# dawn-search/dawnsearch

Measured on NVIDIA B200. Metric: queries/sec, exact top-k over N x 384 fp16, higher is better.
Workload: dtype s8 x s8 -> s32 filter on an int8 shadow (tensor cores) / f32 scan, exact f32 re-score over the fp16 rows

## Files before the change

dawnsearch_b200/csrc/dawn_common.cuh:

```cuda
#pragma once

#include <cuda_fp16.h>
#include <cuda_runtime.h>
#include <stdint.h>

namespace dawn {

constexpr int kDim = 384;
constexpr int kRowBytesF16 = kDim * 2;
constexpr int kMaxCand = 128;
constexpr int kI8BlockRows = 8;
constexpr int kI8BlockBytes = kI8BlockRows * kDim + kI8BlockRows * 4;
constexpr uint32_t kNoRow = 0xFFFFFFFFu;
constexpr uint64_t kNoLabel = 0xFFFFFFFFFFFFFFFFull;

struct __align__(16) Cand {
    float score;
    uint32_t row;
    uint64_t label;
};

__host__ __device__ inline Cand empty_cand() {
    Cand c;
#ifdef __CUDA_ARCH__
    c.score = __int_as_float(0xff800000);
#else
    c.score = -__builtin_inff();
#endif
    c.row = kNoRow;
    c.label = kNoLabel;
    return c;
}

__host__ __device__ inline bool cand_better(const Cand &a, const Cand &b) {
    if (a.score != b.score) return a.score > b.score;
    if (a.label != b.label) return a.label < b.label;
    return a.row < b.row;
}

__device__ inline uint32_t float_to_ordered(float f) {
    uint32_t u = __float_as_uint(f);
    return (u & 0x80000000u) ? ~u : (u | 0x80000000u);
}
__device__ inline float ordered_to_float(uint32_t u) {
    return __uint_as_float((u & 0x80000000u) ? (u & 0x7FFFFFFFu) : ~u);
}

__host__ __device__ inline uint64_t mix64(uint64_t z) {
    z = (z ^ (z >> 30)) * 0xBF58476D1CE4E5B9ull;
    z = (z ^ (z >> 27)) * 0x94D049BB133111EBull;
    return z ^ (z >> 31);
}
__host__ __device__ inline int32_t synth_raw(uint64_t seed, uint64_t row, uint32_t col) {
    uint64_t h = mix64(seed + 0x9E3779B97F4A7C15ull * (row * (uint64_t)kDim + col + 1));
    uint32_t s = (uint32_t)(h & 0xFFFF) + (uint32_t)((h >> 16) & 0xFFFF) +
                 (uint32_t)((h >> 32) & 0xFFFF) + (uint32_t)(h >> 48);
    return (int32_t)s - 131070;
}


cudaError_t launch_ingest_f16(const float *src_f32, __half *dst, size_t n_rows, cudaStream_t s);
cudaError_t launch_synth_f16(__half *dst, uint64_t seed, uint64_t first_row, size_t n_rows,
                             cudaStream_t s);
cudaError_t launch_synth_f32(float *dst, uint64_t seed, uint64_t first_row, size_t n_rows, cudaStream_t s);
cudaError_t launch_gather_f32(const __half *corpus, const uint32_t *rows, size_t n, float *out,
                              cudaStream_t s);
cudaError_t launch_iota_labels(uint64_t *dst, uint64_t first, size_t n, cudaStream_t s);
cudaError_t launch_shadow_quantize(const __half *corpus, uint8_t *arena, size_t first, size_t n, uint32_t *kappa_bits, cudaStream_t s);
cudaError_t launch_truncate_by_limit(const float *dist, uint32_t *counts, size_t batch, size_t k, float limit, cudaStream_t s);

struct ScanLaunch {
    const __half *corpus;
    const uint64_t *labels;
    uint32_t n_rows;
    const float *queries;
    int nq;
    int kprime;
    Cand *partials;
    uint32_t *chunk_counter;
    uint32_t *status;
    int grid;
    float score_floor;
};
cudaError_t launch_scan_topk_f16(const ScanLaunch &p, cudaStream_t s);
int scan_max_queries_per_pass(int kprime);

struct FinalizeLaunch {
    const __half *corpus;
    const float *queries;
    int nq;
    const Cand *partials;
    int n_lists;
    int kprime;
    int k;
    float eps;
    uint64_t *labels_out;
    float *distances_out;
    uint32_t *counts_out;
    uint32_t *flags_out;
    int scalar;
    const float *corpus32;
    const float *eps_q;
    const uint32_t *overflow;
    uint32_t *counters;
    int n_counters;
    uint32_t *status_out;
    float eps_scale;
    uint32_t *stats;
};
cudaError_t launch_score_error(const uint2 *log, const uint32_t *cnt, int n_queries, int log_cap, const __half *corpus,
                               const float *q32, const __half *q16, const float *eps_q, unsigned long long *out,
                               cudaStream_t s);
cudaError_t launch_finalize(const FinalizeLaunch &p, cudaStream_t s);

struct __align__(16) I8Query {
    int8_t hi[kDim];
    int8_t lo[kDim];
    float s1, s2;
    float pad_[2];
};
__host__ __device__ inline size_t i8_row_offset(size_t row) {
// ... 90 lines not shown
```

dawnsearch_b200/csrc/dawn_index.cu:

```cuda
#include <atomic>
#include <cmath>
#include <cstdarg>
#include <cstdio>
#include <cstdlib>
#include <cstring>
#include <chrono>
#include <condition_variable>
#include <mutex>
#include <new>
#include <shared_mutex>
#include <string>
#include <thread>
#include <vector>

#include "../../include/dawn_index.h"
#include "dawn_common.cuh"

using namespace dawn;

namespace {

thread_local std::string g_last_error;

int fail(int code, const char *fmt, ...) {
// ... 72 lines not shown
    std::shared_mutex corpus_mu;
    int device = 0;
    int sm_count = 0;
    cudaStream_t stream = nullptr;
    std::atomic<bool> dead{false};

    int scalar = DAWN_SCALAR_F16;
    __half *corpus = nullptr;
    float *corpus32 = nullptr;
    uint64_t *labels = nullptr;
    std::atomic<uint8_t *> shadow{nullptr};
    std::atomic<size_t> shadow_rows{0};
    std::atomic<float> shadow_kappa{0.f};
    uint32_t *d_shadow_kappa = nullptr;
    std::atomic<size_t> size{0};
    std::atomic<size_t> capacity{0};
    size_t phys = 0;

    float *h_stage_buf[2] = {nullptr, nullptr};
    uint64_t *h_labels_buf[2] = {nullptr, nullptr};
    float *d_stage_buf[2] = {nullptr, nullptr};
    cudaEvent_t stage_done[2] = {nullptr, nullptr};
    bool stage_busy[2] = {false, false};
    int stage_cur = 0;
    float *h_stage = nullptr;
    uint64_t *h_stage_labels = nullptr;
    std::atomic<size_t> staged{0};
    float *d_stage = nullptr;
    BulkLane bulk[kBulkThreads];
    bool bulk_ready = false;

    uint32_t *d_norm_stats = nullptr;
    uint32_t *h_norm_stats = nullptr;
    size_t norm_checked = 0;
    uint64_t bad_rows = 0;
    float norm_max = 0.f, norm_min = INFINITY;

    uint32_t *d_stats = nullptr;
    uint32_t *h_stats = nullptr;

    std::atomic<int64_t> gemm_min_batch{16};
    std::atomic<int64_t> gemm_min_rows{65536};
    std::atomic<int64_t> gemm_small_batch{2};
    std::atomic<int64_t> gemm_small_batch_rows{2000000};
    std::atomic<int64_t> force_path{0};
    std::atomic<int64_t> gemm_cta_group{0};
    std::atomic<int64_t> gemm_chunk_tiles{0};
    std::atomic<int64_t> gemm_sequential_tiles{0};
    std::atomic<int64_t> gemm_growth{0};
    std::atomic<int64_t> gemm_unit_sync{1};
    std::atomic<int64_t> i8_tensor_min_batch{16};
    std::atomic<int64_t> i8_tensor_chunk_rows{4 << 20};
    std::atomic<int64_t> shadow_i8{0};
    std::atomic<int64_t> shadow_big_k_rows{40000000};
    std::atomic<int64_t> shadow_single_rows{6000000};
    std::atomic<int64_t> i8_native{1};

    std::mutex pool_mu;
    std::condition_variable pool_cv;
    std::vector<SearchWs *> pool_free;
    int pool_total = 0;
    std::mutex dev_mu;
    SearchWs *dev_ws = nullptr;

    std::atomic<bool> profiling{false};
    std::mutex prof_mu;
    dawn_profile prof{};
};

namespace {

#define CK(idx, expr)                                                                         \
    do {                                                                                      \
        cudaError_t e__ = (expr);                                                             \
        if (e__ != cudaSuccess) {                                                             \
            (idx)->dead = true;                                                               \
            return fail(DAWN_ERR_CUDA, "%s failed: %s (%s:%d)", #expr, cudaGetErrorString(e__), \
                        __FILE__, __LINE__);                                                  \
        }                                                                                     \
    } while (0)

int check_alive(dawn_index *idx) {
    if (!idx) return fail(DAWN_ERR_INVALID, "null index handle");
    if (idx->dead) return fail(DAWN_ERR_CUDA, "index is in a failed state after an earlier CUDA error");
    cudaError_t e = cudaSetDevice(idx->device);
    if (e != cudaSuccess) {
        idx->dead = true;
        return fail(DAWN_ERR_CUDA, "cudaSetDevice(%d): %s", idx->device, cudaGetErrorString(e));
    }
    return DAWN_OK;
}


void free_ws(SearchWs *ws) {
    if (!ws) return;
    if (ws->stream) cudaStreamSynchronize(ws->stream);
    for (auto &p : ws->pending) ws->free_events.push_back(p);
    for (auto &p : ws->free_events) {
        cudaEventDestroy(p.a);
        cudaEventDestroy(p.b);
    }
    cudaFree(ws->d_queries);
    cudaFreeHost(ws->h_queries);
    cudaFree(ws->d_result);
    cudaFreeHost(ws->h_result);
    cudaFree(ws->d_i8_scratch);
// ... 239 lines not shown
    if (idx->norm_checked >= n) return DAWN_OK;
    CK(idx, launch_verify_rows(idx->corpus, idx->scalar == DAWN_SCALAR_I8 ? 1 : 0, idx->norm_checked, n - idx->norm_checked, idx->d_norm_stats, idx->stream));
    CK(idx, cudaMemcpyAsync(idx->h_norm_stats, idx->d_norm_stats, 4 * sizeof(uint32_t), cudaMemcpyDeviceToHost, idx->stream));
    CK(idx, cudaStreamSynchronize(idx->stream));
    idx->bad_rows = idx->h_norm_stats[0];
    memcpy(&idx->norm_max, &idx->h_norm_stats[1], 4);
    uint32_t inv = ~idx->h_norm_stats[2];
    memcpy(&idx->norm_min, &inv, 4);
    idx->norm_checked = n;
    return DAWN_OK;
}

inline float eps_scale_of(const dawn_index *idx) {
    return idx->norm_max > kRowNormGate ? idx->norm_max / 1.01f * 1.001f : 1.0f;
}

void reset_norm_stats(dawn_index *idx) {
    const uint32_t init[4] = {0u, 0u, 0u, 0u};
    cudaMemcpyAsync(idx->d_norm_stats, init, sizeof init, cudaMemcpyHostToDevice, idx->stream);
    cudaStreamSynchronize(idx->stream);
    idx->norm_checked = 0;
    idx->bad_rows = 0;
    idx->norm_max = 0.f;
    idx->norm_min = INFINITY;
}

void drop_shadow(dawn_index *idx) {
    uint8_t *p = idx->shadow.exchange(nullptr);
    if (p) cudaFree(p);
    idx->shadow_rows = 0;
    idx->shadow_kappa = 0.f;
}

int ensure_shadow(dawn_index *idx) {
    if (!idx->shadow_i8 || idx->scalar != DAWN_SCALAR_F16) return DAWN_OK;
    const size_t n = idx->size;
    if (n < 65536 || idx->shadow_rows >= n) return DAWN_OK;
    if (!idx->shadow) {
        const size_t bytes = (idx->phys + kI8BlockRows - 1) / kI8BlockRows * (size_t)kI8BlockBytes;
        uint8_t *p = nullptr;
        if (cudaMalloc(&p, bytes) != cudaSuccess || (!idx->d_shadow_kappa && cudaMalloc(&idx->d_shadow_kappa, 4) != cudaSuccess)) {
            cudaGetLastError();
            if (p) cudaFree(p);
            idx->shadow_i8 = 0;
            return DAWN_OK;
        }
        CK(idx, cudaMemsetAsync(p, 0, bytes, idx->stream));
        CK(idx, cudaMemsetAsync(idx->d_shadow_kappa, 0, 4, idx->stream));
        idx->shadow = p;
        idx->shadow_rows = 0;
        idx->shadow_kappa = 0.f;
    }
    const size_t first = idx->shadow_rows;
    CK(idx, launch_shadow_quantize(idx->corpus, idx->shadow, first, n - first, idx->d_shadow_kappa, idx->stream));
    uint32_t bits = 0;
    CK(idx, cudaMemcpyAsync(&bits, idx->d_shadow_kappa, 4, cudaMemcpyDeviceToHost, idx->stream));
    CK(idx, cudaStreamSynchronize(idx->stream));
    float kappa;
    memcpy(&kappa, &bits, 4);
    idx->shadow_kappa = kappa * 1.0001f + 1e-4f;
    idx->shadow_rows = n;
    return DAWN_OK;
}

bool debug_stages() {
    static const bool on = getenv("DAWN_DEBUG_STAGES") != nullptr;
    return on;
}
void debug_wait(SearchWs *ws, cudaStream_t s, const char *stage) {
    if (!debug_stages()) return;
    const auto t0 = std::chrono::steady_clock::now();
    while (true) {
        cudaError_t e = cudaStreamQuery(s);
        if (e == cudaSuccess) {
            fprintf(stderr, "[dawn debug] %s done\n", stage);
            return;
        }
        if (e != cudaErrorNotReady) {
            fprintf(stderr, "[dawn debug] %s: %s\n", stage, cudaGetErrorString(e));
            return;
        }
        if (std::chrono::duration<double>(std::chrono::steady_clock::now() - t0).count() > 5.0) {
            uint32_t c[4] = {0, 0, 0, 0};
            cudaStream_t side;
            cudaStreamCreateWithFlags(&side, cudaStreamNonBlocking);
            if (ws->d_counters) {
                cudaMemcpyAsync(c, ws->d_counters, sizeof(c), cudaMemcpyDeviceToHost, side);
                cudaStreamSynchronize(side);
            }
            fprintf(stderr, "[dawn debug] %s STILL RUNNING after 5 s (rows %zu, counters %u %u %u %u)\n", stage, ws->n_rows, c[0],
                    c[1], c[2], c[3]);
            fflush(stderr);
            return;
        }
    }
}

int choose_kprime(size_t k) {
    size_t want = k + (k / 8 > 4 ? k / 8 : 4);
    int kp = 16;
    while ((size_t)kp < want) kp <<= 1;
    return kp > kMaxCand ? kMaxCand : kp;
}

struct ResultView {
    uint64_t *labels;
    float *dist;
// ... 1207 lines not shown
    gs.final_lists = nullptr;
    gs.accum_slack = kGemmAccumSlack;
    gs.limit_score = -INFINITY;
    gs.debug_raw_scores = 1;
    const float *eps_q = nullptr;
    const uint2 *log = nullptr;
    const uint32_t *cnt = nullptr;
    const __half *q16 = nullptr;
    gs.eps_out = &eps_q;
    gs.debug_log_out = &log;
    gs.debug_cnt_out = &cnt;
    gs.debug_q16_out = &q16;
    CK(idx, launch_gemm_search(gs, s));
    unsigned long long *d_out = nullptr;
    CK(idx, cudaMalloc(&d_out, 48 * sizeof(unsigned long long)));
    CK(idx, cudaMemsetAsync(d_out, 0, 48 * sizeof(unsigned long long), s));
    CK(idx, launch_score_error(log, cnt, (int)batch, 2048, idx->corpus, ws->d_queries, q16, eps_q, d_out, s));
    unsigned long long h[48];
    CK(idx, cudaMemcpyAsync(h, d_out, sizeof h, cudaMemcpyDeviceToHost, s));
    CK(idx, cudaStreamSynchronize(s));
    cudaFree(d_out);
    auto as_double = [](unsigned long long u) { double d; memcpy(&d, &u, 8); return d; };
    auto upd = [](double &a, double b) { if (b > a) a = b; };
    upd(acc->max_mma_vs_f64, as_double(h[0]));
    upd(acc->max_seq_vs_f64, as_double(h[1]));
    upd(acc->max_mma_vs_seq, as_double(h[2]));
    upd(acc->max_err_over_eps_q, as_double(h[3]));
    acc->pairs += h[4];
    for (int b = 0; b < 40; b++) acc->hist[b] += h[8 + b];
    acc->scan_eps = kScanEps;
    acc->gemm_accum_slack = kGemmAccumSlack;
    acc->i8_dequant_slack = kI8DequantSlack;
    return DAWN_OK;
}

int dawn_index_set_option(dawn_index *idx, const char *key, int64_t value) {
    int rc = check_alive(idx);
    if (rc) return rc;
    if (!key) return fail(DAWN_ERR_INVALID, "key is null");
    if (!strcmp(key, "gemm_min_batch")) idx->gemm_min_batch = value;
    else if (!strcmp(key, "gemm_min_rows")) idx->gemm_min_rows = value;
    else if (!strcmp(key, "gemm_small_batch")) idx->gemm_small_batch = value;
    else if (!strcmp(key, "gemm_small_batch_rows")) idx->gemm_small_batch_rows = value;
    else if (!strcmp(key, "force_path")) idx->force_path = value;
    else if (!strcmp(key, "gemm_cta_group")) idx->gemm_cta_group = value;
    else if (!strcmp(key, "gemm_chunk_tiles")) idx->gemm_chunk_tiles = value;
    else if (!strcmp(key, "gemm_sequential_tiles")) idx->gemm_sequential_tiles = value;
    else if (!strcmp(key, "gemm_growth")) idx->gemm_growth = value;
    else if (!strcmp(key, "gemm_unit_sync")) idx->gemm_unit_sync = value;
    else if (!strcmp(key, "i8_tensor_min_batch")) idx->i8_tensor_min_batch = value;
    else if (!strcmp(key, "i8_tensor_chunk_rows")) idx->i8_tensor_chunk_rows = value < 65536 ? 65536 : value;
    else if (!strcmp(key, "i8_native")) idx->i8_native = value;
    else if (!strcmp(key, "shadow_i8")) idx->shadow_i8 = value;
    else if (!strcmp(key, "shadow_single_rows")) idx->shadow_single_rows = value;
    else if (!strcmp(key, "shadow_big_k_rows")) idx->shadow_big_k_rows = value;
    else return fail(DAWN_ERR_INVALID, "unknown option '%s'", key);
    return DAWN_OK;
}

int dawn_index_set_profiling(dawn_index *idx, int enable) {
    int rc = check_alive(idx);
    if (rc) return rc;
    {
        std::lock_guard<std::mutex> lk(idx->dev_mu);
        drain_events(idx->dev_ws, idx->dev_ws->ws_used ? idx->dev_ws->ws_stream : idx->dev_ws->stream);
        merge_profile(idx, idx->dev_ws);
    }
    idx->profiling = enable != 0;
    return DAWN_OK;
}

int dawn_index_get_profile(dawn_index *idx, dawn_profile *out, int reset) {
    int rc = check_alive(idx);
    if (rc) return rc;
    if (!out) return fail(DAWN_ERR_INVALID, "out is null");
    {
        std::lock_guard<std::mutex> lk(idx->dev_mu);
        SearchWs *ws = idx->dev_ws;
        cudaStream_t s = ws->ws_used ? ws->ws_stream : ws->stream;
        drain_events(ws, s);
        merge_profile(idx, ws);
        if (ws->ws_used) CK(idx, cudaEventSynchronize(ws->ws_done));
        CK(idx, cudaMemcpy(idx->h_stats, idx->d_stats, 4 * sizeof(uint32_t), cudaMemcpyDeviceToHost));
        if (reset) CK(idx, cudaMemset(idx->d_stats, 0, 4 * sizeof(uint32_t)));
    }
    std::lock_guard<std::mutex> lk(idx->prof_mu);
    *out = idx->prof;
    out->device_uncertified = idx->h_stats[0];
    out->device_status = idx->h_stats[1];
    {
        float e;
        memcpy(&e, &idx->h_stats[2], 4);
        out->max_selection_error = e;
    }
    if (reset) idx->prof = dawn_profile{};
    return DAWN_OK;
}

int dawn_merge_results_device(int device, const uint64_t *d_labels, const float *d_distances,
                              const uint32_t *d_counts, size_t n_lists, size_t list_stride_bytes,
                              size_t batch, size_t k, uint64_t *d_labels_out, float *d_distances_out,
                              uint32_t *d_counts_out, void *stream) {
    if (!d_labels || !d_distances || !d_counts || !d_labels_out || !d_distances_out || !d_counts_out)
        return fail(DAWN_ERR_INVALID, "null device pointer");
    if (k == 0 || k > DAWN_MAX_K || n_lists == 0 || n_lists * k > 1024)
        return fail(DAWN_ERR_INVALID, "merge shape out of range (n_lists=%zu k=%zu; n_lists*k must be <= 1024)",
// ... 163 lines not shown
        if (finite) {
            vmax = fmaxf(vmax, len);
            vmin = fminf(vmin, len);
        }
    }
    if (lane == 0) {
        if (bad) atomicAdd(&stats[0], bad);
        atomicMax(&stats[1], __float_as_uint(vmax));
        atomicMax(&stats[2], ~__float_as_uint(vmin));
    }
}

__global__ void __launch_bounds__(256) iota_labels_kernel(uint64_t *__restrict__ dst, uint64_t first, size_t n) {
    size_t stride = (size_t)gridDim.x * blockDim.x;
    for (size_t i = (size_t)blockIdx.x * blockDim.x + threadIdx.x; i < n; i += stride) dst[i] = first + i;
}

cudaError_t launch_merge_results(const uint64_t *labels, const float *dist, const uint32_t *counts, int n_lists,
                                 size_t list_stride_bytes, int batch, int k, uint64_t *labels_out, float *dist_out,
                                 uint32_t *counts_out, cudaStream_t s) {
    if (n_lists > 64) return cudaErrorInvalidValue;
    size_t sl = list_stride_bytes, sd = list_stride_bytes, sc = list_stride_bytes;
    if (list_stride_bytes == 0) {
        sl = (size_t)batch * k * sizeof(uint64_t);
        sd = (size_t)batch * k * sizeof(float);
        sc = (size_t)batch * sizeof(uint32_t);
    }
    merge_results_kernel<<<batch, 1024, 0, s>>>(labels, dist, counts, n_lists, sl, sd, sc, batch, k, labels_out,
                                                dist_out, counts_out);
    return cudaGetLastError();
}

cudaError_t launch_find_label(const uint64_t *labels, size_t n, uint64_t label, uint32_t *row_out,
                              cudaStream_t s) {
    cudaError_t e = cudaMemsetAsync(row_out, 0xFF, sizeof(uint32_t), s);
    if (e != cudaSuccess) return e;
    size_t blocks = (n + 255) / 256;
    if (blocks > 148 * 8) blocks = 148 * 8;
    find_label_kernel<<<(unsigned)blocks, 256, 0, s>>>(labels, n, label, row_out);
    return cudaGetLastError();
}

cudaError_t launch_verify_rows(const void *arena, int scalar, size_t first, size_t n, uint32_t *stats, cudaStream_t s) {
    if (n == 0) return cudaSuccess;
    size_t blocks = (n + 7) / 8;
    if (blocks > 148 * 8) blocks = 148 * 8;
    verify_rows_kernel<<<(unsigned)blocks, 256, 0, s>>>(static_cast<const uint8_t *>(arena), scalar, first, n, stats);
    return cudaGetLastError();
}

}

namespace dawn {
__global__ void __launch_bounds__(256) shadow_quantize_kernel(const __half *__restrict__ corpus, uint8_t *__restrict__ arena,
                                                              size_t first, size_t n, uint32_t *__restrict__ kappa_bits) {
    const int lane = threadIdx.x & 31;
    const size_t warps = (size_t)gridDim.x * (blockDim.x >> 5);
    float kmax = 0.f;
    for (size_t r = (size_t)blockIdx.x * (blockDim.x >> 5) + (threadIdx.x >> 5); r < n; r += warps) {
        const size_t row = first + r;
        const uint2 *src = reinterpret_cast<const uint2 *>(corpus + row * kDim) + lane * 3;
        float x[12];
        float amax = 0.f;
#pragma unroll
        for (int j = 0; j < 3; j++) {
            const uint2 u = __ldg(src + j);
            const __half2 *h = reinterpret_cast<const __half2 *>(&u);
            const float2 a = __half22float2(h[0]), b = __half22float2(h[1]);
            x[4 * j] = a.x, x[4 * j + 1] = a.y, x[4 * j + 2] = b.x, x[4 * j + 3] = b.y;
        }
#pragma unroll
        for (int j = 0; j < 12; j++) amax = fmaxf(amax, fabsf(x[j]));
#pragma unroll
        for (int off = 16; off > 0; off >>= 1) amax = fmaxf(amax, __shfl_xor_sync(0xffffffffu, amax, off));
        if (!(amax < INFINITY)) amax = 0.f;
        const float sc = amax > 0.f ? __fdiv_rn(amax, 127.0f) : 1.0f;
        uint32_t packed[3];
        float err2 = 0.f;
#pragma unroll
        for (int j = 0; j < 3; j++) {
            uint32_t w = 0;
#pragma unroll
            for (int e = 0; e < 4; e++) {
                const float v = amax > 0.f ? x[4 * j + e] : 0.f;
                const float t = __fdiv_rn(v, sc);
                const int qv = max(-127, min(127, (int)rintf(t)));
                const float d = t - (float)qv;
                err2 = fmaf(d, d, err2);
                w |= ((uint32_t)(qv & 0xff)) << (8 * e);
            }
            packed[j] = w;
        }
#pragma unroll
        for (int off = 16; off > 0; off >>= 1) err2 += __shfl_xor_sync(0xffffffffu, err2, off);
        uint32_t *dst = reinterpret_cast<uint32_t *>(arena + i8_row_offset((uint32_t)row)) + lane * 3;
        dst[0] = packed[0], dst[1] = packed[1], dst[2] = packed[2];
        if (lane == 0) *reinterpret_cast<float *>(arena + i8_scale_offset((uint32_t)row)) = sc;
        kmax = fmaxf(kmax, sqrtf(err2) * 1.00001f);
    }
    if (lane == 0 && kmax > 0.f) atomicMax(kappa_bits, __float_as_uint(kmax));
}

cudaError_t launch_shadow_quantize(const __half *corpus, uint8_t *arena, size_t first, size_t n, uint32_t *kappa_bits,
                                   cudaStream_t s) {
    if (n == 0) return cudaSuccess;
    size_t blocks = (n + 7) / 8;
    if (blocks > 148 * 32) blocks = 148 * 32;
    shadow_quantize_kernel<<<(unsigned)blocks, 256, 0, s>>>(corpus, arena, first, n, kappa_bits);
    return cudaGetLastError();
}

__global__ void truncate_by_limit_kernel(const float *__restrict__ dist, uint32_t *__restrict__ counts, int batch, int k,
                                         float limit) {
    const int b = blockIdx.x * blockDim.x + threadIdx.x;
    if (b >= batch) return;
    const uint32_t c = counts[b];
    uint32_t keep = 0;
    while (keep < c && dist[(size_t)b * k + keep] < limit) keep++;
    counts[b] = keep;
}

cudaError_t launch_truncate_by_limit(const float *dist, uint32_t *counts, size_t batch, size_t k, float limit, cudaStream_t s) {
    truncate_by_limit_kernel<<<(unsigned)((batch + 127) / 128), 128, 0, s>>>(dist, counts, (int)batch, (int)k, limit);
    return cudaGetLastError();
}

cudaError_t launch_iota_labels(uint64_t *dst, uint64_t first, size_t n, cudaStream_t s) {
    if (n == 0) return cudaSuccess;
    size_t blocks = (n + 255) / 256;
    if (blocks > 148 * 8) blocks = 148 * 8;
    iota_labels_kernel<<<(unsigned)blocks, 256, 0, s>>>(dst, first, n);
    return cudaGetLastError();
}
}
```

dawnsearch_b200/csrc/gemm_i8.cu:

```cuda
#include <cuda.h>

#include <cmath>

#include "dawn_common.cuh"
#include "gemm_pipe.cuh"

namespace dawn {

namespace {

using namespace pipe;

constexpr int kI8Threads = 384;
constexpr int BM = 128;
constexpr int BN = 256;
constexpr int BKB = 128;
constexpr int kKBlocks = kDim / BKB;
constexpr int kUmmaKBytes = 32;
constexpr int kRingTiles32K = 4;
constexpr int kMaxStagesB = 2 * kRingTiles32K;
constexpr int kBRingBytes = kRingTiles32K * BN * BKB;
constexpr int kABlockBytes = BM * BKB;
constexpr int kABytes = kABlockBytes * kKBlocks;
constexpr int kTmemCols = 512;
constexpr int kEpiWarps = 8;
constexpr int kEpiThreads = kEpiWarps * 32;
constexpr int kStageCap = 16;
constexpr int kStagingBytes = kStageCap * kEpiThreads * 8;
constexpr int kScaleSlots = 8;
constexpr int kScaleTileBytes = BN * 4;
constexpr int kBarBytes = 512;
constexpr int kGroupMaxBytes = kEpiWarps * 32 * 4;
constexpr int kSmemBytes = 1024 + kABytes + kBRingBytes + kBarBytes + kScaleSlots * kScaleTileBytes + kStagingBytes + kGroupMaxBytes;

__host__ __device__ constexpr uint32_t make_idesc_i8(int m) {
    return (2u << 4) | (1u << 7) | (1u << 10) | ((uint32_t)(BN >> 3) << 17) | ((uint32_t)(m >> 4) << 24);
}

struct I8Smem {
    static constexpr int a_off = 0;
    static constexpr int b_off = kABytes;
    static constexpr int bar_off = kABytes + kBRingBytes;
    static constexpr int scale_off = bar_off + kBarBytes;
    static constexpr int staging_off = scale_off + kScaleSlots * kScaleTileBytes;
    static constexpr int groupmax_off = staging_off + kStagingBytes;
};

__device__ __noinline__ void flush_staged_i8(uint32_t stage_smem, int col, uint32_t n, uint2 *__restrict__ log_q,
                                             uint32_t *__restrict__ cnt_q, uint32_t *__restrict__ overflow_q, int cap) {
    uint32_t slot = atomicAdd(cnt_q, n);
    for (uint32_t e = 0; e < n; e++, slot++) {
        uint2 val;
        asm volatile("ld.shared.v2.u32 {%0, %1}, [%2];" : "=r"(val.x), "=r"(val.y) : "r"(stage_smem + (e * kEpiThreads + col) * 8));
        if (slot < (uint32_t)cap) log_q[slot] = val;
        else *overflow_q = 1u;
    }
}

template <int CG>
__global__ void __launch_bounds__(kI8Threads, 1)
gemm_i8_topk_kernel(const __grid_constant__ CUtensorMap tmap_q, const __grid_constant__ CUtensorMap tmap_x,
                    const __grid_constant__ CUtensorMap tmap_s, uint32_t tile_begin, uint32_t tile_end, uint32_t n_rows,
                    uint32_t n_tiles_total, uint32_t perm_mult, int n_qtiles, int n_queries, int chunk_tiles,
                    const float *__restrict__ thr_g, uint32_t *__restrict__ cnt_g, uint2 *__restrict__ log_g,
                    uint32_t *__restrict__ overflow_g, int log_cap, uint32_t *__restrict__ chunk_arrive,
                    const float *__restrict__ cq_g) {
    constexpr int kStagesB = kRingTiles32K * CG;
    constexpr int kBRows = BN / CG;
    constexpr int kBStageBytes = kBRows * BKB;
    constexpr uint32_t kIdesc = make_idesc_i8(BM * CG);
    extern __shared__ uint8_t smem_raw[];
    const uint32_t base = (smem_u32(smem_raw) + 1023u) & ~1023u;
    const uint32_t a_smem = base + I8Smem::a_off;
    const uint32_t b_smem = base + I8Smem::b_off;
    const uint32_t bars = base + I8Smem::bar_off;
    const uint32_t scale_smem = base + I8Smem::scale_off;
    auto full_bar = [&](int s) { return bars + 8 * s; };
    auto empty_bar = [&](int s) { return bars + 8 * (kMaxStagesB + s); };
    auto tfull_bar = [&](int a) { return bars + 8 * (2 * kMaxStagesB + a); };
    auto tempty_bar = [&](int a) { return bars + 8 * (2 * kMaxStagesB + 2 + a); };
    const uint32_t a_full_bar = bars + 8 * (2 * kMaxStagesB + 4);
    const uint32_t a_free_bar = bars + 8 * (2 * kMaxStagesB + 5);
    auto sfull_bar = [&](int s) { return bars + 8 * (2 * kMaxStagesB + 6 + s); };
    const uint32_t tmem_ptr_smem = bars + 8 * (2 * kMaxStagesB + 6 + kScaleSlots);

    const int warp = threadIdx.x >> 5;
    const int lane = threadIdx.x & 31;
    const uint32_t cta_rank = CG == 2 ? cluster_ctarank() : 0u;
    const uint32_t unit_first = blockIdx.x / CG;
    const uint32_t unit_stride = gridDim.x / CG;

    if (threadIdx.x == 0) {
        for (int s = 0; s < kStagesB; s++) {
            mbar_init(full_bar(s), 1);
            mbar_init(empty_bar(s), 1);
        }
        for (int a = 0; a < 2; a++) {
            mbar_init(tfull_bar(a), 1);
            mbar_init(tempty_bar(a), kEpiWarps * CG);
// ... 81 lines not shown
    } else if (warp == 1 && lane == 0 && cta_rank == 0) {
        uint32_t g = 0, tile_ctr = 0, a_loads = 0;
        int cur_t = -1;
        for (uint32_t u = unit_first; u < n_units; u += unit_stride) {
            const int t = (int)(u % (uint32_t)n_qtiles);
            const uint32_t chunk = u / (uint32_t)n_qtiles;
            if (t != cur_t) {
                mbar_wait(a_full_bar, a_loads & 1u);
                a_loads++;
                cur_t = t;
            }
            const uint32_t tile0 = chunk * chunk_tiles;
            const uint32_t tile1 = min(n_tiles, tile0 + chunk_tiles);
            for (uint32_t tile = tile0; tile < tile1; tile++, tile_ctr++) {
                const uint32_t acc = tile_ctr & 1u;
                mbar_wait(tempty_bar(acc), ((tile_ctr >> 1) & 1u) ^ 1u);
                tc_fence_after();
                const uint32_t d_tmem = tmem_base + acc * BN;
                for (int kb = 0; kb < kKBlocks; kb++, g++) {
                    const uint32_t s = g % kStagesB;
                    mbar_wait(full_bar(s), (g / kStagesB) & 1u);
                    tc_fence_after();
                    const uint64_t adesc = make_kmajor_sw128_desc(a_smem + kb * kABlockBytes);
                    const uint64_t bdesc = make_kmajor_sw128_desc(b_smem + s * kBStageBytes);
#pragma unroll
                    for (int k = 0; k < BKB / kUmmaKBytes; k++) {
                        if constexpr (CG == 2)
                            tc_mma_i8_pair(d_tmem, adesc + (uint64_t)(2 * k), bdesc + (uint64_t)(2 * k), kIdesc,
                                           (uint32_t)((kb | k) != 0));
                        else
                            tc_mma_i8(d_tmem, adesc + (uint64_t)(2 * k), bdesc + (uint64_t)(2 * k), kIdesc,
                                      (uint32_t)((kb | k) != 0));
                    }
                    if constexpr (CG == 2) tc_commit_pair(empty_bar(s));
                    else tc_commit(empty_bar(s));
                }
                if constexpr (CG == 2) tc_commit_pair(tfull_bar(acc));
                else tc_commit(tfull_bar(acc));
            }
            const uint32_t u_next = u + unit_stride;
            if (u_next < n_units && (int)(u_next % (uint32_t)n_qtiles) != t) {
                if constexpr (CG == 2) tc_commit_pair(a_free_bar);
                else tc_commit(a_free_bar);
            }
        }
    } else if (warp >= 4) {
        const int quarter = warp & 3;
        const int half = (warp - 4) >> 2;
        const int col = (warp - 4) * 32 + lane;
        const uint32_t stage_smem = base + I8Smem::staging_off;
        const uint32_t gmax_smem = base + I8Smem::groupmax_off + (uint32_t)(warp - 4) * 128u;
        uint32_t n_st = 0;
        uint32_t tile_ctr = 0;
        const uint32_t tempty_lead0 = CG == 2 ? mapa_rank(tempty_bar(0), 0) : 0u;
        const uint32_t tempty_lead1 = CG == 2 ? mapa_rank(tempty_bar(1), 0) : 0u;
        for (uint32_t u = unit_first; u < n_units; u += unit_stride) {
            const int t = (int)(u % (uint32_t)n_qtiles);
            const uint32_t chunk = u / (uint32_t)n_qtiles;
            const int q = t * BM * CG + (int)cta_rank * BM + quarter * 32 + lane;
            const bool q_valid = q < n_queries;
            const float thr = q_valid ? thr_g[q] : __int_as_float(0x7f800000);
            const float cq = q_valid ? cq_g[q] : 0.0f;
            const bool thr_pos = thr > 0.0f;
            uint2 *log_q = log_g + (size_t)q * log_cap;
            const uint32_t tile0 = chunk * chunk_tiles;
            const uint32_t tile1 = min(n_tiles, tile0 + chunk_tiles);
            uint32_t pt = phys_tile(tile0);
            for (uint32_t tile = tile0; tile < tile1; tile++, tile_ctr++, pt = phys_next(pt)) {
                const uint32_t acc = tile_ctr & 1u;
                const uint32_t row0 = pt * (uint32_t)BN;
                const uint32_t sl = tile_ctr % kScaleSlots;
                const uint32_t sc_addr = scale_smem + sl * kScaleTileBytes + half * (BN / 2) * 4;
                mbar_wait(sfull_bar(sl), (tile_ctr / kScaleSlots) & 1u);
                float smax;
                {
                    float4 s4;
                    asm volatile("ld.shared.v4.f32 {%0, %1, %2, %3}, [%4];"
                                 : "=f"(s4.x), "=f"(s4.y), "=f"(s4.z), "=f"(s4.w)
                                 : "r"(sc_addr + (uint32_t)lane * 16u));
                    smax = fmaxf(fmaxf(s4.x, s4.y), fmaxf(s4.z, s4.w));
                    asm volatile("st.shared.f32 [%0], %1;" ::"r"(gmax_smem + (uint32_t)lane * 4u), "f"(smax) : "memory");
                    smax = fmaxf(smax, __shfl_xor_sync(0xffffffffu, smax, 1));
                    smax = fmaxf(smax, __shfl_xor_sync(0xffffffffu, smax, 2));
                    smax = fmaxf(smax, __shfl_xor_sync(0xffffffffu, smax, 4));
                    __syncwarp();
                }
                mbar_wait(tfull_bar(acc), (tile_ctr >> 1) & 1u);
                tc_fence_after();
                const uint32_t taddr = tmem_base + ((uint32_t)(quarter * 32) << 16) + acc * BN + half * (BN / 2);
                const int lim_tile = (int)n_rows - (int)row0 - half * (BN / 2);
                auto examine = [&](const uint32_t (&v)[32], const int (&m)[8], int c) {
                    float gs[8];
                    asm volatile("ld.shared.v4.f32 {%0, %1, %2, %3}, [%4];"
                                 : "=f"(gs[0]), "=f"(gs[1]), "=f"(gs[2]), "=f"(gs[3])
                                 : "r"(gmax_smem + (uint32_t)c * 32u));
                    asm volatile("ld.shared.v4.f32 {%0, %1, %2, %3}, [%4];"
                                 : "=f"(gs[4]), "=f"(gs[5]), "=f"(gs[6]), "=f"(gs[7])
                                 : "r"(gmax_smem + (uint32_t)c * 32u + 16u));
#pragma unroll
                    for (int g = 0; g < 8; g++) {
                        if (thr_pos && !((__int2float_rn(m[g]) + cq) * gs[g] >= thr)) continue;
                        float4 s4;
                        asm volatile("ld.shared.v4.f32 {%0, %1, %2, %3}, [%4];"
                                     : "=f"(s4.x), "=f"(s4.y), "=f"(s4.z), "=f"(s4.w)
                                     : "r"(sc_addr + (uint32_t)(c * 32 + g * 4) * 4u));
                        const float sc[4] = {s4.x, s4.y, s4.z, s4.w};
#pragma unroll
                        for (int j = 0; j < 4; j++) {
                            const int i = 4 * g + j;
                            const float f = (__int2float_rn((int)v[i]) + cq) * sc[j];
                            if (f >= thr && c * 32 + i < lim_tile) {
                                asm volatile("st.shared.v2.u32 [%0], {%1, %2};" ::"r"(stage_smem + (n_st * kEpiThreads + col) * 8),
                                             "r"(__float_as_uint(f)), "r"(row0 + half * (BN / 2) + c * 32 + i)
                                             : "memory");
                                if (++n_st == (uint32_t)kStageCap) {
                                    flush_staged_i8(stage_smem, col, n_st, log_q, cnt_g + q, overflow_g + q, log_cap);
                                    n_st = 0;
                                }
                            }
                        }
                    }
                };
                auto process = [&](const uint32_t (&v)[32], int c) {
                    int m[8];
#pragma unroll
                    for (int g = 0; g < 8; g++)
                        m[g] = max(max((int)v[4 * g], (int)v[4 * g + 1]), max((int)v[4 * g + 2], (int)v[4 * g + 3]));
                    const int mm = max(max(max(m[0], m[1]), max(m[2], m[3])), max(max(m[4], m[5]), max(m[6], m[7])));
                    const float sm_c = __shfl_sync(0xffffffffu, smax, 8 * c);
                    const bool hit = q_valid && (!thr_pos || (__int2float_rn(mm) + cq) * sm_c >= thr);
                    if (hit) examine(v, m, c);
                    __syncwarp();
                };
                uint32_t v0[32], v1[32];
                tc_ld_32x32b_x32(taddr, v0);
#pragma unroll 1
                for (int c = 0; c < BN / 2 / 32; c += 2) {
                    tc_wait_ld();
                    tc_ld_32x32b_x32(taddr + (c + 1) * 32, v1);
                    process(v0, c);
                    tc_wait_ld();
                    if (c + 2 < BN / 2 / 32) tc_ld_32x32b_x32(taddr + (c + 2) * 32, v0);
                    process(v1, c + 1);
                }
                tc_fence_before();
                __syncwarp();
                if (lane == 0) {
                    if constexpr (CG == 2) mbar_arrive_cluster(acc ? tempty_lead1 : tempty_lead0);
                    else mbar_arrive(tempty_bar(acc));
                }
                if (__any_sync(0xffffffffu, n_st >= (uint32_t)(kStageCap / 2))) {
                    if (n_st) flush_staged_i8(stage_smem, col, n_st, log_q, cnt_g + q, overflow_g + q, log_cap);
                    n_st = 0;
                    __syncwarp();
                }
            }
            if (n_st) {
                flush_staged_i8(stage_smem, col, n_st, log_q, cnt_g + q, overflow_g + q, log_cap);
                n_st = 0;
            }
            __syncwarp();
        }
    }

    tc_fence_before();
    if constexpr (CG == 2) cluster_sync_all();
    else __syncthreads();
    if (warp == 1) {
        tc_fence_after();
        __syncwarp();
        if constexpr (CG == 2)
            asm volatile("tcgen05.dealloc.cta_group::2.sync.aligned.b32 %0, %1;" ::"r"(tmem_base), "r"((uint32_t)kTmemCols));
        else
            asm volatile("tcgen05.dealloc.cta_group::1.sync.aligned.b32 %0, %1;" ::"r"(tmem_base), "r"((uint32_t)kTmemCols));
    }
}

__global__ void __launch_bounds__(128) prep_queries_i8_gemm_kernel(const float *__restrict__ q32, int n_queries,
                                                                   int8_t *__restrict__ q8, float *__restrict__ s1_g,
                                                                   float *__restrict__ e1_g, float *__restrict__ cq_g,
                                                                   float kappa) {
    const int q = blockIdx.x;
    __shared__ float red[4];
    __shared__ float red2[4];
    float x[3], amax = 0.f;
#pragma unroll
    for (int j = 0; j < 3; j++) {
        x[j] = q < n_queries ? q32[(size_t)q * kDim + threadIdx.x + 128 * j] : 0.f;
        amax = fmaxf(amax, fabsf(x[j]));
    }
#pragma unroll
    for (int off = 16; off > 0; off >>= 1) amax = fmaxf(amax, __shfl_xor_sync(0xffffffffu, amax, off));
    if ((threadIdx.x & 31) == 0) red[threadIdx.x >> 5] = amax;
    __syncthreads();
    amax = fmaxf(fmaxf(red[0], red[1]), fmaxf(red[2], red[3]));
    const float s1 = amax > 0.f ? amax / 127.0f : 1.0f;
    float err2 = 0.f, n2 = 0.f;
#pragma unroll
    for (int j = 0; j < 3; j++) {
        const int hi = max(-127, min(127, (int)rintf(x[j] / s1)));
        const float e = fmaf(-s1, (float)hi, x[j]);
        err2 += e * e;
        n2 = fmaf(x[j], x[j], n2);
        q8[(size_t)q * kDim + threadIdx.x + 128 * j] = (int8_t)hi;
    }
#pragma unroll
    for (int off = 16; off > 0; off >>= 1) {
        err2 += __shfl_xor_sync(0xffffffffu, err2, off);
        n2 += __shfl_xor_sync(0xffffffffu, n2, off);
    }
    __syncthreads();
    if ((threadIdx.x & 31) == 0) {
        red[threadIdx.x >> 5] = err2;
        red2[threadIdx.x >> 5] = n2;
    }
// ... 322 lines not shown
    uint32_t *arrive = (n_qtiles > 1 && !p.no_unit_sync) ? reinterpret_cast<uint32_t *>(w + (size_t)qp * kSelCap * sizeof(uint2)) : nullptr;

    static bool configured[64] = {};
    int dev = 0;
    cudaGetDevice(&dev);
    if (dev < 64 && !configured[dev]) {
        cudaError_t e = cudaFuncSetAttribute(gemm_i8_topk_kernel<1>, cudaFuncAttributeMaxDynamicSharedMemorySize, kSmemBytes);
        if (e == cudaSuccess)
            e = cudaFuncSetAttribute(gemm_i8_topk_kernel<2>, cudaFuncAttributeMaxDynamicSharedMemorySize, kSmemBytes);
        if (e != cudaSuccess) return e;
        configured[dev] = true;
    }
    const uint64_t n_blocks = (p.n_rows + kI8BlockRows - 1) / kI8BlockRows;
    CUtensorMap tq, tx, ts;
    if (!make_tmap_q8(&tq, q8, (uint64_t)qp) || !make_tmap_arena(&tx, p.arena, n_blocks, (uint32_t)(BN / cg / kI8BlockRows)) ||
        !make_tmap_scales(&ts, p.arena, n_blocks))
        return cudaErrorInvalidValue;

    cudaError_t e;
    if ((e = cudaMemsetAsync(cnt, 0, (size_t)qp * 3 * sizeof(uint32_t), s)) != cudaSuccess) return e;
    const float kappa = p.rescore_f16 ? p.shadow_kappa : 0.0f;
    if (p.rescore_f16 && !(kappa > 0.0f)) return cudaErrorInvalidValue;
    prep_queries_i8_gemm_kernel<<<qp, 128, 0, s>>>(p.queries, p.n_queries, q8, s1, e1, cq, kappa);
    select_i8_kernel<<<qp, kSelThreads, 0, s>>>(log, cnt, kept, thr, overflow, kSelCap, p.kprime, p.arena, p.queries,
                                                p.n_queries, s1, e1, p.limit_score, p.eps_scale, p.labels, nullptr, arrive,
                                                p.rescore_f16);
    int launches = 2;
    uint64_t growth = p.kprime > 64 ? 4 : 8;
    if (p.growth >= 2) growth = (uint64_t)p.growth;
    const uint64_t band_x4 = p.rescore_f16 ? 22 : 11;
    while (growth > 2 && (growth - 1) * (uint64_t)p.kprime * band_x4 / 4 + (uint64_t)p.kprime > (uint64_t)kSelCap) growth /= 2;
    const uint64_t total_tiles = (p.n_rows + BN - 1) / BN;
    uint64_t mult = (uint64_t)((double)total_tiles * 0.6180339887498949) | 1ull;
    auto gcd = [](uint64_t a, uint64_t b) { while (b) { uint64_t t = a % b; a = b; b = t; } return a; };
    while (mult > 1 && gcd(mult, total_tiles) != 1) mult += 2;
    if (total_tiles <= 2 || p.sequential_tiles) mult = 1;
    mult %= total_tiles > 0 ? total_tiles : 1;
    if (mult == 0) mult = 1;
    uint64_t begin = 0, end = 1024 / BN;
    while (begin < total_tiles) {
        if (end > total_tiles || end + end / 4 > total_tiles) end = total_tiles;
        const uint64_t n_tiles = end - begin;
        uint64_t chunk = (n_tiles * (uint64_t)n_qtiles + (uint64_t)workers * 4 - 1) / ((uint64_t)workers * 4);
        if (chunk < 1) chunk = 1;
        if (chunk > 64) chunk = 64;
        if (p.chunk_tiles > 0) chunk = (uint64_t)p.chunk_tiles;
        if (cg == 2)
            e = launch_round<2>(p.grid, s, tq, tx, ts, (uint32_t)begin, (uint32_t)end, (uint32_t)p.n_rows, (uint32_t)total_tiles,
                                (uint32_t)mult, n_qtiles, p.n_queries, (int)chunk, thr, cnt, log, overflow, arrive, cq);
        else
            e = launch_round<1>(p.grid, s, tq, tx, ts, (uint32_t)begin, (uint32_t)end, (uint32_t)p.n_rows, (uint32_t)total_tiles,
                                (uint32_t)mult, n_qtiles, p.n_queries, (int)chunk, thr, cnt, log, overflow, arrive, cq);
        if (e != cudaSuccess) return e;
        const bool last = end >= total_tiles;
        select_i8_kernel<<<qp, kSelThreads, 0, s>>>(log, cnt, kept, thr, overflow, kSelCap, p.kprime, p.arena, p.queries,
                                                    p.n_queries, s1, e1, p.limit_score, p.eps_scale, p.labels,
                                                    last ? p.final_lists : nullptr, arrive, p.rescore_f16);
        launches += 2;
        begin = end;
        end = end * growth;
    }
    if ((e = cudaGetLastError()) != cudaSuccess) return e;
    if (p.overflow_out) *p.overflow_out = overflow;
    if (p.launches_out) *p.launches_out = launches;
    return cudaSuccess;
}

}
```

Measured before the change: 30110.

## Quantize int8 shadow with shared per-32-row group scale

The shadow quantizer now processes 32-row groups per block and, by default, uses one max-abs scale across the group instead of a per-row scale. The likely aim is that rows in a tile share a scale, so the tensor-core filter's per-group max bound is tighter and fewer warp chunks fall onto the slow examine path. A new option switches between per-row and group scaling and rebuilds the shadow when changed. Compile-time counters for slow-path hits are also added for profiling. Group scaling costs some quantization precision per row, which may raise kappa and loosen the filter.

```diff
diff --git a/dawnsearch_b200/csrc/dawn_common.cuh b/dawnsearch_b200/csrc/dawn_common.cuh
--- a/dawnsearch_b200/csrc/dawn_common.cuh
+++ b/dawnsearch_b200/csrc/dawn_common.cuh
@@ -66,7 +66,8 @@
 cudaError_t launch_gather_f32(const __half *corpus, const uint32_t *rows, size_t n, float *out,
                               cudaStream_t s);
 cudaError_t launch_iota_labels(uint64_t *dst, uint64_t first, size_t n, cudaStream_t s);
-cudaError_t launch_shadow_quantize(const __half *corpus, uint8_t *arena, size_t first, size_t n, uint32_t *kappa_bits, cudaStream_t s);
+cudaError_t launch_shadow_quantize(const __half *corpus, uint8_t *arena, size_t first, size_t n, int group_rows,
+                                   uint32_t *kappa_bits, cudaStream_t s);
 cudaError_t launch_truncate_by_limit(const float *dist, uint32_t *counts, size_t batch, size_t k, float limit, cudaStream_t s);
 
 struct ScanLaunch {
diff --git a/dawnsearch_b200/csrc/dawn_index.cu b/dawnsearch_b200/csrc/dawn_index.cu
--- a/dawnsearch_b200/csrc/dawn_index.cu
+++ b/dawnsearch_b200/csrc/dawn_index.cu
@@ -148,6 +148,7 @@
     std::atomic<int64_t> i8_tensor_min_batch{16};
     std::atomic<int64_t> i8_tensor_chunk_rows{4 << 20};
     std::atomic<int64_t> shadow_i8{0};
+    std::atomic<int64_t> shadow_group_rows{32};
     std::atomic<int64_t> shadow_big_k_rows{40000000};
     std::atomic<int64_t> shadow_single_rows{6000000};
     std::atomic<int64_t> i8_native{1};
@@ -493,7 +494,8 @@
         idx->shadow_kappa = 0.f;
     }
     const size_t first = idx->shadow_rows;
-    CK(idx, launch_shadow_quantize(idx->corpus, idx->shadow, first, n - first, idx->d_shadow_kappa, idx->stream));
+    CK(idx, launch_shadow_quantize(idx->corpus, idx->shadow, first, n - first, (int)idx->shadow_group_rows, idx->d_shadow_kappa,
+                                   idx->stream));
     uint32_t bits = 0;
     CK(idx, cudaMemcpyAsync(&bits, idx->d_shadow_kappa, 4, cudaMemcpyDeviceToHost, idx->stream));
     CK(idx, cudaStreamSynchronize(idx->stream));
@@ -1807,6 +1809,16 @@
     else if (!strcmp(key, "i8_tensor_chunk_rows")) idx->i8_tensor_chunk_rows = value < 65536 ? 65536 : value;
     else if (!strcmp(key, "i8_native")) idx->i8_native = value;
     else if (!strcmp(key, "shadow_i8")) idx->shadow_i8 = value;
+    else if (!strcmp(key, "shadow_group_rows")) {
+        if (value != 1 && value != 32) return fail(DAWN_ERR_INVALID, "shadow_group_rows must be 1 or 32, not %lld", (long long)value);
+        std::lock_guard<std::mutex> lk(idx->mu);
+        if (idx->shadow_group_rows != value) {
+            std::unique_lock<std::shared_mutex> wr(idx->corpus_mu);
+            wait_device_searches(idx);
+            drop_shadow(idx);
+            idx->shadow_group_rows = value;
+        }
+    }
     else if (!strcmp(key, "shadow_single_rows")) idx->shadow_single_rows = value;
     else if (!strcmp(key, "shadow_big_k_rows")) idx->shadow_big_k_rows = value;
     else return fail(DAWN_ERR_INVALID, "unknown option '%s'", key);
@@ -2076,61 +2088,92 @@
 }
 
 namespace dawn {
+constexpr int kShadowGroupRows = 32;
 __global__ void __launch_bounds__(256) shadow_quantize_kernel(const __half *__restrict__ corpus, uint8_t *__restrict__ arena,
-                                                              size_t first, size_t n, uint32_t *__restrict__ kappa_bits) {
-    const int lane = threadIdx.x & 31;
-    const size_t warps = (size_t)gridDim.x * (blockDim.x >> 5);
+                                                              size_t first, size_t n, int group_rows,
+                                                              uint32_t *__restrict__ kappa_bits) {
+    __shared__ float s_amax[8];
+    const int lane = threadIdx.x & 31, warp = threadIdx.x >> 5;
+    const size_t end = first + n;
+    const size_t g_end = (end + kShadowGroupRows - 1) / kShadowGroupRows;
     float kmax = 0.f;
-    for (size_t r = (size_t)blockIdx.x * (blockDim.x >> 5) + (threadIdx.x >> 5); r < n; r += warps) {
-        const size_t row = first + r;
-        const uint2 *src = reinterpret_cast<const uint2 *>(corpus + row * kDim) + lane * 3;
-        float x[12];
-        float amax = 0.f;
+    for (size_t g = first / kShadowGroupRows + blockIdx.x; g < g_end; g += gridDim.x) {
+        float amax[4], wmax = 0.f;
 #pragma unroll
-        for (int j = 0; j < 3; j++) {
-            const uint2 u = __ldg(src + j);
-            const __half2 *h = reinterpret_cast<const __half2 *>(&u);
-            const float2 a = __half22float2(h[0]), b = __half22float2(h[1]);
-            x[4 * j] = a.x, x[4 * j + 1] = a.y, x[4 * j + 2] = b.x, x[4 * j + 3] = b.y;
-        }
+        for (int i = 0; i < 4; i++) {
+            const size_t row = g * kShadowGroupRows + warp + 8 * i;
+            float m = 0.f;
+            if (row >= first && row < end) {
+                const uint2 *src = reinterpret_cast<const uint2 *>(corpus + row * kDim) + lane * 3;
 #pragma unroll
-        for (int j = 0; j < 12; j++) amax = fmaxf(amax, fabsf(x[j]));
+                for (int j = 0; j < 3; j++) {
+                    const uint2 u = __ldg(src + j);
+                    const float2 a = __half22float2(*reinterpret_cast<const __half2 *>(&u.x));
+                    const float2 b = __half22float2(*reinterpret_cast<const __half2 *>(&u.y));
+                    m = fmaxf(fmaxf(m, fmaxf(fabsf(a.x), fabsf(a.y))), fmaxf(fabsf(b.x), fabsf(b.y)));
+                }
+            }
 #pragma unroll
-        for (int off = 16; off > 0; off >>= 1) amax = fmaxf(amax, __shfl_xor_sync(0xffffffffu, amax, off));
-        if (!(amax < INFINITY)) amax = 0.f;
-        const float sc = amax > 0.f ? __fdiv_rn(amax, 127.0f) : 1.0f;
-        uint32_t packed[3];
-        float err2 = 0.f;
+            for (int off = 16; off > 0; off >>= 1) m = fmaxf(m, __shfl_xor_sync(0xffffffffu, m, off));
+            if (!(m < INFINITY)) m = 0.f;
+            amax[i] = m;
+            wmax = fmaxf(wmax, m);
+        }
+        if (group_rows > 1) {
+            if (lane == 0) s_amax[warp] = wmax;
+            __syncthreads();
+            wmax = s_amax[0];
 #pragma unroll
-        for (int j = 0; j < 3; j++) {
-            uint32_t w = 0;
+            for (int w = 1; w < 8; w++) wmax = fmaxf(wmax, s_amax[w]);
+            __syncthreads();
+        }
+#pragma unroll 1
+        for (int i = 0; i < 4; i++) {
+            const size_t row = g * kShadowGroupRows + warp + 8 * i;
+            if (row < first || row >= end) continue;
+            const float ra = i == 0 ? amax[0] : i == 1 ? amax[1] : i == 2 ? amax[2] : amax[3];
+            const float m = group_rows > 1 ? wmax : ra;
+            const float sc = m > 0.f ? __fdiv_rn(m, 127.0f) : 1.0f;
+            const uint2 *src = reinterpret_cast<const uint2 *>(corpus + row * kDim) + lane * 3;
+            uint32_t packed[3];
+            float err2 = 0.f;
 #pragma unroll
-            for (int e = 0; e < 4; e++) {
-                const float v = amax > 0.f ? x[4 * j + e] : 0.f;
-                const float t = __fdiv_rn(v, sc);
-                const int qv = max(-127, min(127, (int)rintf(t)));
-                const float d = t - (float)qv;
-                err2 = fmaf(d, d, err2);
-                w |= ((uint32_t)(qv & 0xff)) << (8 * e);
+            for (int j = 0; j < 3; j++) {
+                const uint2 u = __ldg(src + j);
+                const float2 a = __half22float2(*reinterpret_cast<const __half2 *>(&u.x));
+                const float2 b = __half22float2(*reinterpret_cast<const __half2 *>(&u.y));
+                const float xs[4] = {a.x, a.y, b.x, b.y};
+                uint32_t w = 0;
+#pragma unroll
+                for (int e = 0; e < 4; e++) {
+                    const float v = ra > 0.f ? xs[e] : 0.f;
+                    const float t = __fdiv_rn(v, sc);
+                    const int qv = max(-127, min(127, (int)rintf(t)));
+                    const float d = t - (float)qv;
+                    err2 = fmaf(d, d, err2);
+                    w |= ((uint32_t)(qv & 0xff)) << (8 * e);
+                }
+                packed[j] = w;
             }
-            packed[j] = w;
-        }
 #pragma unroll
-        for (int off = 16; off > 0; off >>= 1) err2 += __shfl_xor_sync(0xffffffffu, err2, off);
-        uint32_t *dst = reinterpret_cast<uint32_t *>(arena + i8_row_offset((uint32_t)row)) + lane * 3;
-        dst[0] = packed[0], dst[1] = packed[1], dst[2] = packed[2];
-        if (lane == 0) *reinterpret_cast<float *>(arena + i8_scale_offset((uint32_t)row)) = sc;
-        kmax = fmaxf(kmax, sqrtf(err2) * 1.00001f);
+            for (int off = 16; off > 0; off >>= 1) err2 += __shfl_xor_sync(0xffffffffu, err2, off);
+            uint32_t *dst = reinterpret_cast<uint32_t *>(arena + i8_row_offset((uint32_t)row)) + lane * 3;
+            dst[0] = packed[0], dst[1] = packed[1], dst[2] = packed[2];
+            if (lane == 0) *reinterpret_cast<float *>(arena + i8_scale_offset((uint32_t)row)) = sc;
+            kmax = fmaxf(kmax, sqrtf(err2) * 1.00001f);
+        }
     }
     if (lane == 0 && kmax > 0.f) atomicMax(kappa_bits, __float_as_uint(kmax));
 }
 
-cudaError_t launch_shadow_quantize(const __half *corpus, uint8_t *arena, size_t first, size_t n, uint32_t *kappa_bits,
-                                   cudaStream_t s) {
+cudaError_t launch_shadow_quantize(const __half *corpus, uint8_t *arena, size_t first, size_t n, int group_rows,
+                                   uint32_t *kappa_bits, cudaStream_t s) {
     if (n == 0) return cudaSuccess;
-    size_t blocks = (n + 7) / 8;
-    if (blocks > 148 * 32) blocks = 148 * 32;
-    shadow_quantize_kernel<<<(unsigned)blocks, 256, 0, s>>>(corpus, arena, first, n, kappa_bits);
+    if (group_rows != 1 && group_rows != kShadowGroupRows) return cudaErrorInvalidValue;
+    const size_t groups = (first + n + kShadowGroupRows - 1) / kShadowGroupRows - first / kShadowGroupRows;
+    size_t blocks = groups;
+    if (blocks > 148 * 8) blocks = 148 * 8;
+    shadow_quantize_kernel<<<(unsigned)blocks, 256, 0, s>>>(corpus, arena, first, n, group_rows, kappa_bits);
     return cudaGetLastError();
 }
 
diff --git a/dawnsearch_b200/csrc/gemm_i8.cu b/dawnsearch_b200/csrc/gemm_i8.cu
--- a/dawnsearch_b200/csrc/gemm_i8.cu
+++ b/dawnsearch_b200/csrc/gemm_i8.cu
@@ -45,6 +45,24 @@
     static constexpr int staging_off = scale_off + kScaleSlots * kScaleTileBytes;
     static constexpr int groupmax_off = staging_off + kStagingBytes;
 };
+
+#ifdef DAWN_COUNT_SLOW_PATH
+__device__ unsigned long long g_slow_acc[2];
+constexpr int kSlowLogCap = 4096;
+__device__ unsigned long long g_slow_log[kSlowLogCap][4];
+__device__ unsigned int g_slow_log_n;
+__global__ void slow_path_log_kernel(uint32_t tiles, int n_queries) {
+    const unsigned int i = g_slow_log_n;
+    if (i < (unsigned int)kSlowLogCap) {
+        g_slow_log[i][0] = g_slow_acc[0];
+        g_slow_log[i][1] = g_slow_acc[1];
+        g_slow_log[i][2] = tiles;
+        g_slow_log[i][3] = (unsigned long long)n_queries;
+        g_slow_log_n = i + 1;
+    }
+    g_slow_acc[0] = g_slow_acc[1] = 0ull;
+}
+#endif
 
 __device__ __noinline__ void flush_staged_i8(uint32_t stage_smem, int col, uint32_t n, uint2 *__restrict__ log_q,
                                              uint32_t *__restrict__ cnt_q, uint32_t *__restrict__ overflow_q, int cap) {
@@ -232,6 +250,9 @@
         const uint32_t gmax_smem = base + I8Smem::groupmax_off + (uint32_t)(warp - 4) * 128u;
         uint32_t n_st = 0;
         uint32_t tile_ctr = 0;
+#ifdef DAWN_COUNT_SLOW_PATH
+        uint32_t n_slow = 0, n_wchunks = 0;
+#endif
         const uint32_t tempty_lead0 = CG == 2 ? mapa_rank(tempty_bar(0), 0) : 0u;
         const uint32_t tempty_lead1 = CG == 2 ? mapa_rank(tempty_bar(1), 0) : 0u;
         for (uint32_t u = unit_first; u < n_units; u += unit_stride) {
@@ -309,6 +330,10 @@
                     const int mm = max(max(max(m[0], m[1]), max(m[2], m[3])), max(max(m[4], m[5]), max(m[6], m[7])));
                     const float sm_c = __shfl_sync(0xffffffffu, smax, 8 * c);
                     const bool hit = q_valid && (!thr_pos || (__int2float_rn(mm) + cq) * sm_c >= thr);
+#ifdef DAWN_COUNT_SLOW_PATH
+                    n_slow += __any_sync(0xffffffffu, hit) ? 1u : 0u;
+                    n_wchunks++;
+#endif
                     if (hit) examine(v, m, c);
                     __syncwarp();
                 };
@@ -341,6 +366,12 @@
             }
             __syncwarp();
         }
+#ifdef DAWN_COUNT_SLOW_PATH
+        if (lane == 0) {
+            atomicAdd(&g_slow_acc[0], (unsigned long long)n_slow);
+            atomicAdd(&g_slow_acc[1], (unsigned long long)n_wchunks);
+        }
+#endif
     }
 
     tc_fence_before();
@@ -769,6 +800,9 @@
             e = launch_round<1>(p.grid, s, tq, tx, ts, (uint32_t)begin, (uint32_t)end, (uint32_t)p.n_rows, (uint32_t)total_tiles,
                                 (uint32_t)mult, n_qtiles, p.n_queries, (int)chunk, thr, cnt, log, overflow, arrive, cq);
         if (e != cudaSuccess) return e;
+#ifdef DAWN_COUNT_SLOW_PATH
+        slow_path_log_kernel<<<1, 1, 0, s>>>((uint32_t)(end - begin), p.n_queries);
+#endif
         const bool last = end >= total_tiles;
         select_i8_kernel<<<qp, kSelThreads, 0, s>>>(log, cnt, kept, thr, overflow, kSelCap, p.kprime, p.arena, p.queries,
                                                     p.n_queries, s1, e1, p.limit_score, p.eps_scale, p.labels,
@@ -784,3 +818,17 @@
 }
 
 }
+
+#ifdef DAWN_COUNT_SLOW_PATH
+extern "C" int dawn_debug_slow_path_log(unsigned long long *out, int cap, int reset) {
+    unsigned int n = 0;
+    if (cudaDeviceSynchronize() != cudaSuccess || cudaMemcpyFromSymbol(&n, dawn::g_slow_log_n, sizeof n) != cudaSuccess) return -1;
+    const int m = (int)n < cap ? (int)n : cap;
+    if (m > 0 && cudaMemcpyFromSymbol(out, dawn::g_slow_log, (size_t)m * 4 * sizeof(unsigned long long)) != cudaSuccess) return -1;
+    if (reset) {
+        const unsigned int zero = 0;
+        if (cudaMemcpyToSymbol(dawn::g_slow_log_n, &zero, sizeof zero) != cudaSuccess) return -1;
+    }
+    return (int)n;
+}
+#endif
```

Result: faster. 33540, median of 6 (+11.4%).
